# projectchrono/DEM-Engine

Measured on AMD Instinct MI355X. Metric: clump*steps/s, higher is better.
Workload: dtype f32 physics / f64 geometry

## Files before the change

### dem-engine_amd/csrc/deme_hip.hip

```cpp
#include <algorithm>
#include <cmath>
#include <cstdarg>
#include <cstdio>
#include <cstdlib>
#include <chrono>
#include <cstring>
#include <condition_variable>
#include <functional>
#include <memory>
#include <mutex>
#include <dlfcn.h>
#include <map>
#include <string>
#include <thread>
#include <vector>

#include <hip/hip_runtime.h>
#include <rocprim/rocprim.hpp>
template <unsigned RB, unsigned IPT = 8>
using DemeRadixCfg = rocprim::radix_sort_config<rocprim::default_config, rocprim::default_config,
                                                rocprim::radix_sort_onesweep_config<rocprim::kernel_config<1024, IPT>, rocprim::kernel_config<1024, IPT>, RB,
                                                                                    rocprim::block_radix_rank_algorithm::match>,
                                                1024 * 1024>;
#include <array>
// ... 125 lines not shown
    bool seeded = false;
    hipModule_t prescMod = nullptr;
    hipFunction_t prescFn = nullptr;
    DevBuf prescList, prescSlot, prescRec;
    DevBuf userWc[4][8];
    uint32_t nOwnerWc = 0, nGeoWc = 0;
    bool hasGhosts = false;
    uint32_t asyncLead = 0;
    DevBuf revSlot;
    const void* revAcc = nullptr;
    bool pairsOnce = false;
    PrescArgs laterPa{nullptr, nullptr};
    bool crossStale = false;
    char* pin = nullptr;
    int spinSync = 1;
    bool snapPending = false;
    DevBuf ownersSnap;
    hipStream_t detStream = nullptr;
    hipEvent_t evSnap = nullptr, evP1 = nullptr;
    uint64_t nAsyncDetections = 0;
    std::vector<uint32_t> hShared;
    DevBuf sharedIds, sharedBuf;
    bool tailFused = true;
    bool inGroupStep = false;
    hipStream_t haloStream = nullptr;
    hipEvent_t evStepDone = nullptr, evHaloDone = nullptr;
    bool overlapDetect = false;
    hipModule_t rulesMod = nullptr;
    DemeAdaptive ad{};
    hipEvent_t evDet0 = nullptr, evDet1 = nullptr, evWin0 = nullptr, evWin1 = nullptr;
// ... 67 lines not shown
}

#define HIPCK(call)                                                                                   \
    do {                                                                                              \
        hipError_t _e = (call);                                                                       \
        if (_e != hipSuccess)                                                                         \
            return fail(c, DEME_ERR_HIP, "%s failed: %s (%s:%d)", #call, hipGetErrorString(_e), __FILE__, __LINE__); \
    } while (0)

constexpr size_t PIN_BYTES = 16384;
constexpr size_t PIN_HEAVY = 0;
constexpr size_t PIN_RANGES = 128;
constexpr size_t PIN_LEGACY = 256;
constexpr size_t PIN_TRI = 384;
constexpr size_t PIN_UNIQUE = 448;
constexpr size_t PIN_DETECT = 1024;
static_assert(PIN_HEAVY + sizeof(RangeCounters) <= PIN_RANGES && PIN_RANGES + sizeof(RangeCounters) <= PIN_LEGACY &&
                  PIN_LEGACY + sizeof(RangeCounters) <= PIN_TRI && PIN_TRI + sizeof(uint32_t) <= PIN_UNIQUE &&
                  PIN_UNIQUE + sizeof(unsigned long long) <= PIN_DETECT && PIN_DETECT + sizeof(DetectHead) <= PIN_BYTES,
              "the read-back slots overlap or leave the pinned block");
static_assert(PIN_RANGES % 8 == 0 && PIN_LEGACY % 8 == 0 && PIN_TRI % 8 == 0 && PIN_UNIQUE % 8 == 0 && PIN_DETECT % 8 == 0,
              "a read-back slot is aligned for the counters it holds");
template <typename T>
static inline T* pin_at(deme_ctx* c, size_t slot) {
    return reinterpret_cast<T*>(c->pin + slot);
}
static hipError_t sync_readback(deme_ctx* c, hipStream_t st, bool spin) {
    if (c->spinSync && spin) {
        const auto t0 = std::chrono::steady_clock::now();
        for (int it = 0;; it++) {
            const hipError_t q = hipStreamQuery(st);
            if (q != hipErrorNotReady)
                return q;
            if ((it & 255) == 255 && std::chrono::steady_clock::now() - t0 > std::chrono::milliseconds(5))
                break;
        }
    }
    return hipStreamSynchronize(st);
}
template <typename T>
const T* read_back(deme_ctx* c, size_t slot, const void* dev, hipStream_t st, bool spin, size_t bytes = sizeof(T)) {
    T* host = pin_at<T>(c, slot);
    hipError_t e = hipMemcpyAsync(host, dev, bytes, hipMemcpyDeviceToHost, st);
    if (e == hipSuccess)
        e = sync_readback(c, st, spin);
    if (e == hipSuccess)
        return host;
    fail(c, DEME_ERR_HIP, "a detection's read-back failed: %s", hipGetErrorString(e));
    return nullptr;
}

int ensure(deme_ctx* c, DevBuf& b, size_t bytes, bool keep = false) {
    if (bytes <= b.bytes && b.p)
        return DEME_OK;
    size_t want = std::max<size_t>(bytes, 256);
    if (b.p)
        want = std::max(want, b.bytes + b.bytes / 4);
    void* np = nullptr;
    HIPCK(hipMalloc(&np, want));
    if (keep && b.p && b.bytes)
        HIPCK(hipMemcpyAsync(np, b.p, b.bytes, hipMemcpyDeviceToDevice, c->stream));
    if (b.p) {
        HIPCK(hipStreamSynchronize(c->stream));
        HIPCK(hipFree(b.p));
// ... 265 lines not shown
    return launch_margins(c, c->stream, c->owners.as<OwnerRec>(), drift);
}

int do_migrate(deme_ctx* c);

struct DetectRun {
    hipStream_t st;
    OwnerRec* ow;
    bool async;
    bool statusSeen = false;
    KeyArena ar{};
    bool segmented = false;
    uint32_t P = 0;
    uint32_t nStats = 0, compactBlocks = 0;
    uint64_t raw = 0, segMax = 0;
    DetectCounters hc{};
};
inline unsigned bin_id_bits(const deme_ctx* c) { return bits_for((uint64_t)c->hp.nbX * c->hp.nbY * c->hp.nbZ, 32); }

void open_key_arena(deme_ctx* c, DetectRun& d) {
    DetectBlock* blk = c->ctr.as<DetectBlock>();
    d.segmented = c->keySegMin && c->cntCap >= c->keySegMin && c->cntCap >= DEME_KEY_SEGS * 64u;
    d.ar.keys = c->keysRaw.as<uint64_t>();
    d.ar.segMask = d.segmented ? DEME_KEY_SEGS - 1u : 0u;
    d.ar.segCap = d.segmented ? (uint64_t)c->cntCap / DEME_KEY_SEGS : (uint64_t)c->cntCap;
    d.ar.ctr = d.segmented ? blk->segCtr : &blk->c.nContactsRaw;
}

const DetectHead* read_detect_counters(deme_ctx* c, DetectRun& d, size_t bytes) {
    const DetectHead* hh = read_back<DetectHead>(c, PIN_DETECT, c->ctr.p, d.st, !d.async, bytes);
    if (!hh || (!d.statusSeen && status_to_error(c, hh->c.status & ~DEME_ST_INCIDENCE)))
        return nullptr;
    d.statusSeen = true;
    d.hc = hh->c;
    return hh;
}

int detect_sphere_incidences(deme_ctx* c, DetectRun& d) {
    const uint32_t nS = c->nSpheres;
    d.P = 0;
    auto fill_incidence = [&]() {
        hipLaunchKernelGGL(k_fill_incidence, dim3(grid_for(nS)), dim3(256), 0, d.st, c->dp, c->binLo.as<uint4>(), c->binN.as<uint2>(),
                           c->binPartial.as<uint32_t>(), c->incKeys[0].as<uint32_t>(), c->incVals[0].as<uint32_t>(), (uint64_t)c->incCap);
    };
    if (nS) {
        c->geoStale = false;
        hipLaunchKernelGGL(k_sphere_prep, dim3(grid_for(nS)), dim3(256), 0, d.st, c->dp, d.ow, c->spheres.as<SphereRec>(),
                           c->geo.as<GeoRec>(), c->binLo.as<uint4>(), c->binN.as<uint2>(), c->binPartial.as<uint32_t>(), d.ar,
                           c->ctr.as<DetectCounters>(), c->sphFam.as<uint16_t>());
        hipLaunchKernelGGL(k_scan_small, dim3(1), dim3(DEME_SCAN_T), 0, d.st, c->binPartial.as<uint32_t>(), c->binPartial.as<uint32_t>(),
                           grid_for(nS), &c->ctr.as<DetectBlock>()->c.nIncidence);
        const bool early = c->incCap != 0;
        if (early)
            fill_incidence();
        if (!read_detect_counters(c, d, sizeof(DetectCounters)))
            return c->lastStatus;
        if (d.hc.status & DEME_ST_INCIDENCE)
            return fail(c, DEME_ERR_OVERFLOW,
                        "a sphere touches more than %u bins (margin far larger than the bin size): the incidence list cannot be built",
                        DEME_MAX_BINS_PER_SPHERE);
        if (d.hc.nIncidence > 0xFFFFFFFFull)
            return fail(c, DEME_ERR_OVERFLOW, "%llu bin-sphere incidences do not fit the 32-bit list offsets (use larger bins)",
                        d.hc.nIncidence);
        d.P = (uint32_t)d.hc.nIncidence;
        const bool grow = d.P > c->incCap;
        if (grow)
            if (int rc = grow_incidence_arena(c, (size_t)d.P + d.P / 4 + 1024))
                return rc;
        if (d.P && (grow || !early))
            fill_incidence();
    }
// ... 61 lines not shown
    hipLaunchKernelGGL(k_tri_fill, dim3(grid_for(nT)), dim3(256), 0, st, c->dp, nT, c->triWorld.as<TriWorld>(), c->triLo.as<int4>(),
                       c->triHi.as<int4>(), c->triOffsets.as<uint32_t>(), c->triKeys[0].as<uint32_t>(), c->triVals[0].as<uint32_t>(),
                       (uint64_t)c->triCap);
    if (int rc = with_temp(c, c->sortTmp, [&](void* tmp, size_t& bytes) {
            return rocprim::radix_sort_pairs(tmp, bytes, c->triKeys[0].as<uint32_t>(), c->triKeys[1].as<uint32_t>(),
                                             c->triVals[0].as<uint32_t>(), c->triVals[1].as<uint32_t>(), (size_t)TP, 0, bin_id_bits(c), st);
        }))
        return rc;
    hipLaunchKernelGGL(k_tri_sweep, dim3(grid_for(TP)), dim3(256), 0, st, c->dp, TP, c->triKeys[1].as<uint32_t>(),
                       c->triVals[1].as<uint32_t>(), c->triWorld.as<TriWorld>(), d.P, c->incKeys[1].as<uint32_t>(),
                       c->incVals[1].as<uint32_t>(), c->geo.as<GeoRec>(), c->sphFam.as<uint16_t>(), d.ar);
    return DEME_OK;
}
int detect_close_arena(deme_ctx* c, DetectRun& d) {
    d.compactBlocks = 0;
    if (d.segmented) {
        d.compactBlocks = (uint32_t)std::min<uint64_t>(grid_for(std::max<uint64_t>(c->lastSegMax + c->lastSegMax / 8 + 1024, 1)), grid_for(d.ar.segCap));
        hipLaunchKernelGGL(k_compact_keys, dim3(d.compactBlocks, DEME_KEY_SEGS), dim3(256), 0, d.st, c->keysRaw.as<uint64_t>(), d.ar.segCap,
                           c->ctr.as<DetectBlock>(), 0u, c->keysSorted[c->keysCur ^ 1].as<uint64_t>(), c->binStat.as<uint2>(), d.nStats);
    }
    const DetectHead* hh = read_detect_counters(c, d, d.segmented ? sizeof(DetectHead) : sizeof(DetectCounters));
    if (!hh)
        return c->lastStatus;
    d.raw = d.hc.nContactsRaw, d.segMax = 0;
    if (d.segmented) {
        d.raw = 0;
        for (uint32_t g = 0; g < DEME_KEY_SEGS; g++) {
            d.raw += hh->segCount[g];
            d.segMax = std::max<uint64_t>(d.segMax, hh->segCount[g]);
        }
    }
    return DEME_OK;
}

size_t contact_arena_wanted(uint64_t raw, uint64_t segMax, uint64_t segCap, size_t marks, size_t cap) {
    size_t grow = 0;
    if (raw > cap || segMax > segCap) {
        const size_t want = std::max<size_t>(raw, (size_t)segMax * DEME_KEY_SEGS);
        grow = want + want / 4 + 1024;
    }
    if (marks && raw + marks > std::max(cap, grow))
        grow = (size_t)raw + marks + raw / 4 + 1024;
    return grow;
}

int detect_order_keys(deme_ctx* c, DetectRun& d, uint64_t* nCout) {
    const hipStream_t st = d.st;
    const size_t nPersist = c->hPersist.size();
    uint64_t nC = d.raw + nPersist;
    const int next = c->keysCur ^ 1;
    uint64_t* rawKeys = c->keysRaw.as<uint64_t>();
    if (d.segmented) {
        c->lastSegMax = d.segMax;
        if (grid_for(d.segMax) > d.compactBlocks)
            hipLaunchKernelGGL(k_compact_keys, dim3((unsigned)grid_for(d.segMax) - d.compactBlocks, DEME_KEY_SEGS), dim3(256), 0, st,
                               c->keysRaw.as<uint64_t>(), d.ar.segCap, c->ctr.as<DetectBlock>(), d.compactBlocks,
                               c->keysSorted[next].as<uint64_t>(), (const uint2*)nullptr, 0u);
        if (d.raw)
            rawKeys = c->keysSorted[next].as<uint64_t>();
    }
    if (nPersist)
        HIPCK(hipMemcpyAsync(rawKeys + d.raw, c->persistKeys.p, nPersist * 8, hipMemcpyDeviceToDevice, st));
    if (nC) {
        const unsigned bitsA = bits_for(c->dp.nSpheres, 31);
        if (int rc = ensure(c, c->keysMid, (size_t)c->cntCap * 8))
            return rc;
        uint64_t* mid = c->keysMid.as<uint64_t>();
        if (int rc = with_temp(c, c->sortTmp, [&](void* tmp, size_t& bytes) {
                return deme_radix_sort<DemeRadixCfg<8>, false>(tmp, bytes, rawKeys, mid, nullptr, nullptr, (size_t)nC, (size_t)c->cntCap, 31,
                                                               33 + bitsA, DEME_SORT_OWN_FROM_KEYS64, st);
            }))
            return rc;
// ... 28 lines not shown
        if (int rc = detect_sphere_incidences(c, d))
            return rc;
        if (int rc = detect_sort_sweep(c, d))
            return rc;
        if (int rc = detect_triangles(c, d))
            return rc;
        if (int rc = detect_close_arena(c, d))
            return rc;
        if (const size_t cap = contact_arena_wanted(d.raw, d.segMax, d.ar.segCap, c->hPersist.size(), c->cntCap)) {
            if (async)
                HIPCK(hipStreamSynchronize(c->stream));
            if (int rc = grow_contact_arena(c, cap))
                return rc;
            continue;
        }
        c->nActiveBins = d.hc.nActiveBins;
        c->maxInBin = d.hc.maxInBin ? d.hc.maxInBin : (d.P ? 1u : 0u);
        if (c->maxInBin > c->dp.errOutBinSphNum)
            return fail(c, DEME_ERR_BIN_TOO_FULL,
                        "a bin contains %u sphere components, exceeding the allowance %u (SetMaxSphereInBin)", c->maxInBin,
                        c->dp.errOutBinSphNum);
        return detect_order_keys(c, d, nCout);
    }
    return fail(c, DEME_ERR_OVERFLOW, "contact arena kept overflowing");
}

int build_legacy_lists(deme_ctx* c, ContactList& L, const OwnerRec* ow, hipStream_t st) {
    const uint64_t nC = L.nListed;
    if (nC) {
        const unsigned obits = bits_for(c->nOwners, 32);
        if (int rc = with_temp(c, c->sortTmp, [&](void* tmp, size_t& bytes) {
                return rocprim::radix_sort_pairs(tmp, bytes, L.ownerB[0].as<uint32_t>(), L.ownerB[1].as<uint32_t>(), L.bIdx[0].as<uint32_t>(),
                                                 L.bIdx[1].as<uint32_t>(), (size_t)nC, 0, obits, st);
            }))
            return rc;
    }
    if (c->hasGhosts) {
// ... 80 lines not shown
            unsigned int* cnt = &L.rangeCtr.as<RangeCounters>()->nSM;
            if (int rc = with_temp(c, c->scanTmp, [&](void* tmp, size_t& bytes) {
                    return rocprim::select(tmp, bytes, rocprim::counting_iterator<uint32_t>(0), L.smFlag.as<uint8_t>(), L.smList.as<uint32_t>(), cnt,
                                           (size_t)nC, st);
                }))
                return rc;
        }
        hipLaunchKernelGGL(k_run_starts, dim3(grid_for(nC)), dim3(256), 0, st, (uint32_t)nC, L.ownerA.as<uint32_t>(), c->nOwners,
                           L.aStart.as<uint32_t>());
    } else {
        HIPCK(hipMemsetAsync(L.aStart.p, 0, ((size_t)c->nOwners + 1) * 4, st));
    }
    L.nListed = nC, L.listKeys = next;
    return DEME_OK;
}
int build_tiles(deme_ctx* c, ContactList& L, const OwnerRec* ow, hipStream_t st, RangeCounters& hr) {
    const uint32_t nTiles = tile_count(c);
    hipLaunchKernelGGL(k_scan_small, dim3(1), dim3(DEME_SCAN_T), 0, st, L.tileRem.as<uint32_t>(), L.tileBase.as<uint32_t>(), nTiles + 1,
                       &L.rangeCtr.as<RangeCounters>()->nRemote);
    hipLaunchKernelGGL(k_tile_build, dim3(nTiles), dim3(256), 0, st, c->dp, c->nOwners, L.info.as<uint4>(),
                       L.ownerB[0].as<uint32_t>(), L.aStart.as<uint32_t>(), ow, L.tileBase.as<uint32_t>(), L.tInfo.as<uint2>(),
                       L.hList.as<uint32_t>(), L.hCount.as<uint32_t>(),
                       c->hasGhosts ? L.tileMode.as<uint32_t>() : (uint32_t*)nullptr, L.lOff.as<uint16_t>(),
                       L.lPos.as<uint16_t>(), L.lCount.as<uint32_t>(), L.rankC.as<uint32_t>(), L.remKey[0].as<uint32_t>(),
                       L.remVal.as<uint32_t>(), L.tileOrg.as<int64_t>(), L.rangeCtr.as<RangeCounters>(), nTiles,
                       L.tileBig.as<uint32_t>(), L.bigList.as<uint32_t>(), c->recContact.as<uint32_t>());
    hipLaunchKernelGGL(k_tile_stats, dim3((nTiles + 1023u) / 1024u), dim3(256), 0, st, nTiles, L.hCount.as<uint32_t>(),
                       L.lCount.as<uint32_t>(), L.rangeCtr.as<RangeCounters>());
    const RangeCounters* got = read_back<RangeCounters>(c, PIN_RANGES, L.rangeCtr.p, st, true);
    if (!got)
        return c->lastStatus;
    hr = *got;
    const uint32_t nR = (uint32_t)hr.nRemote + hr.nExtra;
    L.nBigTiles = hr.nBig;
    const unsigned obits = bits_for(c->nOwners, 32);
    if (nR) {
        if (int rc = with_temp(c, c->sortTmp, [&](void* tmp, size_t& bytes) {
                return deme_radix_sort<DemeRadixCfg<10>, true>(tmp, bytes, L.remKey[0].as<uint32_t>(), L.remKey[1].as<uint32_t>(),
                                                               L.remVal.as<uint32_t>(), L.rIdx.as<uint32_t>(), (size_t)nR, (size_t)c->cntCap, 0, obits,
                                                               DEME_SORT_OWN_FROM_RECORDS, st);
            }))
            return rc;
        hipLaunchKernelGGL(k_run_starts, dim3(grid_for(nR)), dim3(256), 0, st, nR, L.remKey[1].as<uint32_t>(), c->nOwners,
                           L.rStart.as<uint32_t>());
    } else {
        HIPCK(hipMemsetAsync(L.rStart.p, 0, ((size_t)c->nOwners + 1) * 4, st));
    }
    hipLaunchKernelGGL(k_owner_ranges_tile, dim3(grid_for(c->nOwners)), dim3(256), 0, st, c->dp, ow, L.aStart.as<uint32_t>(),
                       L.lOff.as<uint16_t>(), L.rStart.as<uint32_t>(), L.heavy.as<uint8_t>(), L.fixedFlag.as<uint8_t>(),
                       L.heavyList.as<uint32_t>(), (uint32_t)(L.heavyList.bytes / 4), L.rangeCtr.as<RangeCounters>());
    return DEME_OK;
}
int build_closed_tiles(deme_ctx* c, ContactList& L, const OwnerRec* ow, hipStream_t st) {
    const uint32_t nTiles = tile_count(c);
    hipLaunchKernelGGL(k_in_count, dim3(grid_for((size_t)c->nOwners + 1)), dim3(256), 0, st, c->dp, ow,
                       L.rStart.as<uint32_t>(), c->inCnt.as<uint32_t>());
    if (int rc = with_temp(c, c->scanTmp, [&](void* tmp, size_t& bytes) {
            return rocprim::exclusive_scan(tmp, bytes, c->inCnt.as<uint32_t>(), c->inStart.as<uint32_t>(), 0u, (size_t)c->nOwners + 1,
                                           rocprim::plus<uint32_t>(), st);
        }))
        return rc;
    hipLaunchKernelGGL(k_tile_incoming, dim3(nTiles), dim3(256), 0, st, c->dp, c->nOwners, L.info.as<uint4>(),
// ... 13 lines not shown
}
void commit_list(deme_ctx* c, uint64_t nC) {
    c->fusedPrevValid = false;
    c->conValid = false;
    c->nPrev = c->haveList ? c->nContacts : 0;
    c->nContacts = nC;
    c->keysCur ^= 1;
    c->listSerial++;
    c->haveList = true;
    c->seeded = false;
    c->mapFresh = true;
    c->nDetections++;
}

void order_watch_drift(deme_ctx* c, const RangeCounters& hr);
int detect_part2(deme_ctx* c, ContactList& L, const OwnerRec* ow, hipStream_t st, uint64_t nC) {
    L.invalidate();
    const bool tiled = tile_eligible(c, nC);
    RangeCounters hr{};
    if (int rc = build_owner_arrays(c, L, st, nC, tiled))
        return rc;
    if (tiled) {
        if (int rc = build_tiles(c, L, ow, st, hr))
            return rc;
        if (fused_eligible(c, hr))
            if (int rc = build_closed_tiles(c, L, ow, st))
                return rc;
        if (int rc = fetch_heavy_counts(c, L, st))
            return rc;
    } else {
        if (int rc = build_legacy_lists(c, L, ow, st))
            return rc;
        if (int rc = read_legacy_counts(c, L, st, hr))
            return rc;
    }
    L.tileActive = tiled;
    L.tileMaxHalo = hr.tileMaxHalo, L.tileMaxList = hr.tileMaxList;
    L.nSA = hr.nSA;
// ... 1 lines not shown
    if (tiled)
        order_watch_drift(c, hr);
    commit_list(c, nC);
    return DEME_OK;
}


int do_detect(deme_ctx* c) {
    if (c->mapFresh)
        if (int rc = do_migrate(c))
            return rc;
    ScopedTimer tm(c, "detect", true);
    uint64_t nC = 0;
    if (int rc = detect_part1(c, c->stream, c->owners.as<OwnerRec>(), false, &nC))
        return rc;
    return detect_part2(c, c->list[c->cur], c->owners.as<OwnerRec>(), c->stream, nC);
}

int do_migrate(deme_ctx* c) {
    ContactList& L = c->list[c->cur];
    const uint32_t nW = c->hp.nContactWildcards;
    if (!c->mapFresh)
        return DEME_OK;
    c->mapFresh = false;
    if (nW == 0) {
        c->nWcStored = c->nContacts;
        return DEME_OK;
    }
    const int next = c->wcCur ^ 1;
    if (c->nContacts)
        hipLaunchKernelGGL(k_migrate, dim3(grid_for(c->nContacts)), dim3(256), 0, c->stream, (uint32_t)c->nContacts, nW,
// ... 415 lines not shown
    deme_ctx* c = new deme_ctx();
    c->device = device;
    if (hipStreamCreateWithFlags(&c->stream, hipStreamNonBlocking) != hipSuccess) {
        delete c;
        return DEME_ERR_HIP;
    }
    if (ensure(c, c->ctr, sizeof(DetectBlock)) || ensure(c, c->scanTmp, 1 << 20)) {
        delete c;
        return DEME_ERR_HIP;
    }
    hipMemsetAsync(c->ctr.p, 0, sizeof(DetectBlock), c->stream);
    if (hipHostMalloc((void**)&c->pin, PIN_BYTES, hipHostMallocDefault) != hipSuccess) {
        deme_ctx_destroy(c);
        return DEME_ERR_HIP;
    }
    if (const char* e = getenv("DEME_ARITH"))
        c->arith = (strcmp(e, "exact") == 0) ? DEME_ARITH_EXACT : DEME_ARITH_FAST;
    if (const char* e = getenv("DEME_XCD_GROUP"))
        c->xcdGroup = (uint32_t)std::max(0, atoi(e));
    if (const char* e = getenv("DEME_SPIN_SYNC"))
        c->spinSync = atoi(e);
    if (const char* e = getenv("DEME_KEY_SEG_MIN"))
        c->keySegMin = (size_t)std::max(0ll, atoll(e));
    *out = c;
    return DEME_OK;
}

void deme_ctx_destroy(deme_ctx* c) {
    if (!c)
        return;
    hipSetDevice(c->device);
    hipStreamSynchronize(c->stream);
    drain_timers(c);
    for (auto e : c->eventPool)
        hipEventDestroy(e);
    for (hipModule_t m : {c->customMod, c->prescMod, c->rulesMod})
// ... 7 lines not shown
            hipEventDestroy(e);
    if (c->haloStream) {
        hipStreamSynchronize(c->haloStream);
        hipEventDestroy(c->evStepDone);
        hipEventDestroy(c->evHaloDone);
        hipStreamDestroy(c->haloStream);
    }
    if (c->pin)
        hipHostFree(c->pin);
    for (ContactList& l : c->list)
        for (DevBuf* b : l.buffers())
            if (b->p)
                hipFree(b->p);
    if (c->hrEvent)
        hipEventDestroy(c->hrEvent);
    if (c->detStream) {
        hipStreamSynchronize(c->detStream);
        hipEventDestroy(c->evSnap);
        hipEventDestroy(c->evP1);
        hipStreamDestroy(c->detStream);
    }
    DevBuf* all[] = {&c->hCountIn, &c->ownersNext, &c->recContact, &c->inCnt, &c->inStart, &c->tInfoIn, &c->inContact,
                     &c->sphFam, &c->dO2E, &c->dS2E, &c->rec32, &c->revSlot, &c->nextAcc, &c->binStat, &c->volumes,
                     &c->persistKeys, &c->owners, &c->spheres, &c->acc, &c->conA4, &c->conA2, &c->conB4, &c->conB2, &c->aSum,
                     &c->prescList, &c->prescSlot, &c->prescRec, &c->tris, &c->triWorld, &c->triLo, &c->triHi, &c->triCounts,
                     &c->triOffsets, &c->triKeys[0], &c->triKeys[1], &c->triVals[0], &c->triVals[1], &c->comp, &c->massProps,
                     &c->anal, &c->matPair, &c->E, &c->nu, &c->CoR, &c->mu, &c->Crr, &c->famMasks, &c->famExtra, &c->famFlags,
                     &c->geo, &c->binLo, &c->binN, &c->binPartial, &c->incKeys[0], &c->incKeys[1], &c->incVals[0],
                     &c->incVals[1], &c->keysRaw, &c->keysSorted[0], &c->keysSorted[1], &c->wc[0], &c->wc[1], &c->ctr,
                     &c->scanTmp, &c->sortTmp, &c->rec[0], &c->rec[1], &c->rec[2], &c->rec[3], &c->stage, &c->sharedIds,
// ... 762 lines not shown
        return DEME_OK;
    if (int rc = ensure(c, c->ownersSnap, (size_t)c->nOwners * sizeof(OwnerRec)))
        return rc;
    if (int rc = ensure(c, c->keysMid, (size_t)c->cntCap * 8))
        return rc;
    return async_size_next(c);
}
static int async_part2(deme_ctx* c, uint64_t nC) {
    ContactList& N = c->list[c->cur ^ 1];
    if (int rc = async_size_next(c))
        return rc;
    {
        ScopedTimer tm(c, "detect_async_part2", true, c->detStream);
        HIPCK(hipMemsetAsync(N.heavy.p, 0, N.heavy.bytes, c->detStream));
        HIPCK(hipMemsetAsync(N.fixedFlag.p, 0, N.fixedFlag.bytes, c->detStream));
        if (int rc = detect_part2(c, N, c->ownersSnap.as<OwnerRec>(), c->detStream, nC))
            return rc;
    }
    c->cur ^= 1;
    HIPCK(hipEventRecord(c->evP1, c->detStream));
    HIPCK(hipStreamWaitEvent(c->stream, c->evP1, 0));
    if (int rc = do_migrate(c))
        return rc;
    c->stepsSinceCD = 0;
    c->listStale = false;
    c->nAsyncDetections++;
    return DEME_OK;
}
static int async_detection_cycle(deme_ctx* c) {
    const uint32_t D = c->asyncLead;
    if (int rc = async_snapshot(c))
// ... 2473 lines not shown
```

### dem-engine_amd/csrc/deme_kernels.h

```cpp
#pragma once
#include "deme_device.h"
#include "deme_owner_cols.h"

namespace deme_dev {

#define DEME_NULL_BINID_DEV 0xFFFFFFFFu
#define DEME_ST_VELOCITY 1u
#define DEME_ST_NONFINITE 2u
#define DEME_ST_INCIDENCE 4u
#define DEME_MAX_BINS_PER_SPHERE 0xFFFFFFu

struct DetectCounters {
    unsigned long long nContactsRaw;
    unsigned int nActiveBins;
    unsigned int maxInBin;
    unsigned int status;
    unsigned int pad0;
    unsigned long long nIncidence;
    unsigned int pad[8];
};

#define DEME_KEY_SEGS 64u
#define DEME_KEY_SEG_STRIDE 16u
struct DetectBlock {
// ... 9 lines not shown
    uint64_t* keys;
    unsigned long long* ctr;
    uint64_t segCap;
    uint32_t segMask;
};
__device__ inline uint32_t arena_seg(const KeyArena& a) {
    return blockIdx.x & a.segMask;
}
__device__ inline unsigned long long arena_reserve(const KeyArena& a, uint32_t seg, unsigned long long n) {
    return atomicAdd(&a.ctr[seg * DEME_KEY_SEG_STRIDE], n);
}
__device__ inline void arena_store(const KeyArena& a, uint32_t seg, unsigned long long slot, uint64_t key) {
    if (slot < a.segCap)
        a.keys[(uint64_t)seg * a.segCap + slot] = key;
}
__device__ void bin_stats_block(const uint2* __restrict__ perBlock, uint32_t nBlocks, uint32_t block, DetectCounters* ctr);
__global__ __launch_bounds__(256) void k_compact_keys(const uint64_t* __restrict__ in, uint64_t segCap, DetectBlock* blk, uint32_t xOff,
                                                      uint64_t* __restrict__ out, const uint2* __restrict__ stats, uint32_t nStats) {
    __shared__ unsigned long long sStart, sCount;
    const uint32_t seg = blockIdx.y;
    if (threadIdx.x < 64) {
        static_assert(DEME_KEY_SEGS == 64, "one lane per segment");
        const unsigned long long raw = blk->segCtr[threadIdx.x * DEME_KEY_SEG_STRIDE];
        if (stats && seg == 0 && blockIdx.x == 0)
            blk->segCount[threadIdx.x] = raw;
        const unsigned long long cnt = min(raw, (unsigned long long)segCap);
        unsigned long long inc = cnt;
        for (int d = 1; d < 64; d <<= 1) {
            const unsigned long long u = __shfl_up(inc, d);
            if ((int)threadIdx.x >= d)
                inc += u;
        }
        if (threadIdx.x == seg)
            sStart = inc - cnt, sCount = cnt;
    }
    __syncthreads();
    const uint64_t i = ((uint64_t)xOff + blockIdx.x) * blockDim.x + threadIdx.x;
    if (i < sCount)
        out[sStart + i] = in[(uint64_t)seg * segCap + i];
    if (stats && seg == 0)
// ... 130 lines not shown
                    unsigned long long slot0 = 0;
                    if ((int)lane == leader)
                        slot0 = arena_reserve(ar, arena_seg(ar), (unsigned long long)__popcll(m));
                    slot0 = __shfl(slot0, leader);
                    const unsigned long long slot = slot0 + (unsigned long long)__popcll(m & ((1ull << lane) - 1ull));
                    if (hit)
                        arena_store(ar, arena_seg(ar), slot, make_key(DEME_KEY_CLASS_SA, s, ob0 + k));
                }
            }
        }
    }
}

#define DEME_SCAN_T 1024u
#define DEME_SCAN_IPT 4u
__global__ __launch_bounds__(DEME_SCAN_T) void k_scan_small(const uint32_t* in, uint32_t* out, uint32_t n, unsigned long long* totalOut) {
    __shared__ unsigned long long sWave[DEME_SCAN_T / 64];
    __shared__ unsigned long long sCarry;
    const uint32_t lane = threadIdx.x & 63u, w = threadIdx.x >> 6;
    if (threadIdx.x == 0)
        sCarry = 0;
    __syncthreads();
    for (uint32_t base = 0; base < n; base += DEME_SCAN_T * DEME_SCAN_IPT) {
        const uint32_t first = base + threadIdx.x * DEME_SCAN_IPT;
        uint32_t v[DEME_SCAN_IPT];
        unsigned long long sum = 0;
#pragma unroll
        for (uint32_t i = 0; i < DEME_SCAN_IPT; i++) {
            v[i] = first + i < n ? in[first + i] : 0u;
            sum += v[i];
        }
// ... 13 lines not shown
            total += t;
        }
#pragma unroll
        for (uint32_t i = 0; i < DEME_SCAN_IPT; i++) {
            if (first + i < n)
                out[first + i] = (uint32_t)run;
            run += v[i];
        }
        __syncthreads();
        if (threadIdx.x == 0)
            sCarry += total;
        __syncthreads();
    }
    if (threadIdx.x == 0)
        *totalOut = sCarry;
}

__global__ __launch_bounds__(256) void k_fill_incidence(const DevParams p, const uint4* __restrict__ binLo,
                                                        const uint2* __restrict__ binN,
                                                        const uint32_t* __restrict__ partialPrefix,
                                                        uint32_t* __restrict__ keys, uint32_t* __restrict__ vals,
                                                        uint64_t cap) {
    __shared__ uint32_t sWaveSum[4];
    const uint32_t s = blockIdx.x * blockDim.x + threadIdx.x;
    const bool valid = s < p.nSpheres;
    const uint4 lo = valid ? binLo[s] : make_uint4(0u, 0u, 0u, 0u);
    const uint2 n = valid ? binN[s] : make_uint2(0u, 0u);
    const uint64_t n64 = (uint64_t)lo.w * n.x * n.y;
    const uint32_t cnt = n64 > DEME_MAX_BINS_PER_SPHERE ? 0u : (uint32_t)n64;
    const uint32_t lane = threadIdx.x & 63u, w = threadIdx.x >> 6;
// ... 854 lines not shown
}

#define DEME_HEAVY_THRESHOLD 256u
struct RangeCounters {
    unsigned int nHeavy;
    unsigned int nHeavyFree;
    unsigned int nSA, nSM;
    unsigned int tileOverflow;
    unsigned int tileMaxHalo, tileMaxList;
    unsigned int nBig;
    unsigned int nExtra;
    unsigned int tileHaloSum;
    unsigned int nBigIn;
    unsigned int tileMaxHaloIn;
    unsigned long long nRemote;
    unsigned int pad[2];
};

__global__ __launch_bounds__(256) void k_run_starts(uint32_t n, const uint32_t* __restrict__ owner, uint32_t nOwners,
                                                    uint32_t* __restrict__ start) {
    const uint32_t i = blockIdx.x * blockDim.x + threadIdx.x;
    if (i >= n)
        return;
    const uint32_t cur = owner[i];
    const uint32_t first = (i == 0) ? 0u : owner[i - 1] + 1u;
    for (uint32_t o = first; o <= cur && o <= nOwners; o++)
        start[o] = i;
    if (i == n - 1)
        for (uint32_t o = cur + 1; o <= nOwners; o++)
            start[o] = n;
}

// ... 462 lines not shown
```

### dem-engine_amd/csrc/deme_tile.h

```cpp
#pragma once
#include "deme_force_fast.h"

#ifndef DEME_TILE_NB
#define DEME_TILE_NB 128
#endif
#ifndef DEME_TILE_HMAX
#define DEME_TILE_HMAX 192
#endif
#ifndef DEME_TILE_T
#define DEME_TILE_T 256
#endif
#define DEME_TILE_HP2 256
#define DEME_TILE_LREG 4
#define DEME_TILE_LMAX (DEME_TILE_LREG * DEME_TILE_T)
static_assert(DEME_TILE_T >= 2 * DEME_TILE_NB, "one pulling thread per owner and side");
static_assert(DEME_TILE_NB + DEME_TILE_HMAX <= 2 * DEME_TILE_T, "a thread stages at most two owner records");
static_assert(DEME_TILE_LMAX == DEME_TILE_LREG * DEME_TILE_T, "list entries per thread");
#define DEME_TILE_HASH 1024u
#ifndef DEME_TILE_REC
#define DEME_TILE_REC 6
#endif
#define DEME_TILE_REC_USER 5
#ifndef DEME_JIT_NW
#define DEME_JIT_NW 1
// ... 925 lines not shown
            while (j > b && lp[j - 1] > v) {
                lp[j] = lp[j - 1];
                j--;
            }
            lp[j] = v;
        }
    }
    __syncthreads();
    for (uint32_t i = tid; i < nLoc; i += 256)
        lPos[c0 + i] = lp[i];
    for (uint32_t i = tid; i <= DEME_TILE_NB; i += 256)
        lOff[(size_t)t * (DEME_TILE_NB + 1) + i] = (uint16_t)off[i];
}

__global__ __launch_bounds__(256) void k_tile_stats(uint32_t nTiles, const uint32_t* __restrict__ hCount,
                                                    const uint32_t* __restrict__ lCount, RangeCounters* rc) {
    __shared__ uint32_t mh[4], ml[4], sh[4];
    uint32_t a = 0, b = 0, sum = 0;
    for (uint32_t k = 0; k < 4; k++) {
        const uint32_t t = (blockIdx.x * 4u + k) * 256u + threadIdx.x;
        if (t < nTiles)
            a = max(a, hCount[t]), b = max(b, lCount[t]), sum += hCount[t];
    }
    for (int o = 32; o > 0; o >>= 1) {
        a = max(a, (uint32_t)__shfl_xor((int)a, o));
        b = max(b, (uint32_t)__shfl_xor((int)b, o));
        sum += (uint32_t)__shfl_xor((int)sum, o);
    }
    if ((threadIdx.x & 63u) == 0)
        mh[threadIdx.x >> 6] = a, ml[threadIdx.x >> 6] = b, sh[threadIdx.x >> 6] = sum;
    __syncthreads();
    if (threadIdx.x == 0) {
        atomicAdd(&rc->tileHaloSum, sh[0] + sh[1] + sh[2] + sh[3]);
        atomicMax(&rc->tileMaxHalo, max(max(mh[0], mh[1]), max(mh[2], mh[3])));
        atomicMax(&rc->tileMaxList, max(max(ml[0], ml[1]), max(ml[2], ml[3])));
    }
}

__global__ __launch_bounds__(256) void k_owner_ranges_tile(const DevParams p, const OwnerRec* __restrict__ owners,
                                                           const uint32_t* __restrict__ aStart, const uint16_t* __restrict__ lOff,
                                                           const uint32_t* __restrict__ rStart, uint8_t* __restrict__ heavy,
                                                           uint8_t* __restrict__ fixedFlag, uint32_t* __restrict__ heavyList,
                                                           uint32_t heavyCap, RangeCounters* rc) {
    const uint32_t o = blockIdx.x * blockDim.x + threadIdx.x;
    if (o >= p.nOwners)
        return;
    const uint32_t t = o / DEME_TILE_NB, k = o - t * DEME_TILE_NB;
    const uint16_t* lo = lOff + (size_t)t * (DEME_TILE_NB + 1);
    const uint32_t nA = aStart[o + 1] - aStart[o], nB = (uint32_t)(lo[k + 1] - lo[k]) + (rStart[o + 1] - rStart[o]);
    const uint32_t fw = owners[o].family;
// ... 19 lines not shown
```

Before: 6.520 billion.

## Post detection counters to pinned host mailboxes instead of stream-sync read-backs

Kernels now write small counter payloads plus a stamped flag straight into pinned host memory (system-scope release stores), and the host spins on that flag instead of issuing a memcpy and synchronizing the stream. It also starts the remote-record sort speculatively from the mailed count when the last detection had no big tiles, and defers the bin-stat read-back behind an event so key ordering can be enqueued first. This is meant to cut host-device round-trip latency on the contact-detection critical path. The cost is more complex ordering logic, a last-block ticket in k_tile_stats, and a fallback path when the mail times out.

```diff
diff --git a/dem-engine_amd/csrc/deme_hip.hip b/dem-engine_amd/csrc/deme_hip.hip
--- a/dem-engine_amd/csrc/deme_hip.hip
+++ b/dem-engine_amd/csrc/deme_hip.hip
@@ -163,6 +163,11 @@
     bool crossStale = false;
     char* pin = nullptr;
     int spinSync = 1;
+    int mailbox = 1;
+    char* pinDev = nullptr;
+    uint32_t mailStamp = 0;
+    hipEvent_t statEvent = nullptr;
+    int lastBigTiles = -1;
     bool snapPending = false;
     DevBuf ownersSnap;
     hipStream_t detStream = nullptr;
@@ -260,13 +265,28 @@
 constexpr size_t PIN_LEGACY = 256;
 constexpr size_t PIN_TRI = 384;
 constexpr size_t PIN_UNIQUE = 448;
+constexpr size_t PIN_BINSTAT = 512;
 constexpr size_t PIN_DETECT = 1024;
+constexpr size_t mail_bytes(size_t payload) { return payload + 8; }
+struct SegCounts {
+    unsigned long long n[DEME_KEY_SEGS];
+};
+constexpr size_t PIN_MAIL_INC = 640;
+constexpr size_t PIN_MAIL_REMOTE = 768;
+constexpr size_t PIN_MAIL_RANGES = 896;
+constexpr size_t PIN_MAIL_KEYS = 2048;
 static_assert(PIN_HEAVY + sizeof(RangeCounters) <= PIN_RANGES && PIN_RANGES + sizeof(RangeCounters) <= PIN_LEGACY &&
                   PIN_LEGACY + sizeof(RangeCounters) <= PIN_TRI && PIN_TRI + sizeof(uint32_t) <= PIN_UNIQUE &&
-                  PIN_UNIQUE + sizeof(unsigned long long) <= PIN_DETECT && PIN_DETECT + sizeof(DetectHead) <= PIN_BYTES,
+                  PIN_UNIQUE + sizeof(unsigned long long) <= PIN_BINSTAT && PIN_BINSTAT + sizeof(DetectCounters) <= PIN_MAIL_INC &&
+                  PIN_MAIL_INC + mail_bytes(8) <= PIN_MAIL_REMOTE && PIN_MAIL_REMOTE + mail_bytes(8) <= PIN_MAIL_RANGES &&
+                  PIN_MAIL_RANGES + mail_bytes(sizeof(RangeCounters)) <= PIN_DETECT && PIN_DETECT + sizeof(DetectHead) <= PIN_MAIL_KEYS &&
+                  PIN_MAIL_KEYS + mail_bytes(sizeof(SegCounts)) <= PIN_BYTES,
               "the read-back slots overlap or leave the pinned block");
-static_assert(PIN_RANGES % 8 == 0 && PIN_LEGACY % 8 == 0 && PIN_TRI % 8 == 0 && PIN_UNIQUE % 8 == 0 && PIN_DETECT % 8 == 0,
+static_assert(PIN_RANGES % 8 == 0 && PIN_LEGACY % 8 == 0 && PIN_TRI % 8 == 0 && PIN_UNIQUE % 8 == 0 && PIN_DETECT % 8 == 0 &&
+                  PIN_BINSTAT % 8 == 0,
               "a read-back slot is aligned for the counters it holds");
+static_assert(PIN_MAIL_INC % 128 == 0 && PIN_MAIL_REMOTE % 128 == 0 && PIN_MAIL_RANGES % 128 == 0 && PIN_MAIL_KEYS % 128 == 0,
+              "a mail slot starts a cache line: the host polls it while copies land in the slots beside it");
 template <typename T>
 static inline T* pin_at(deme_ctx* c, size_t slot) {
     return reinterpret_cast<T*>(c->pin + slot);
@@ -294,6 +314,62 @@
         return host;
     fail(c, DEME_ERR_HIP, "a detection's read-back failed: %s", hipGetErrorString(e));
     return nullptr;
+}
+
+struct MailReq {
+    unsigned long long* dev = nullptr;
+    uint32_t stamp = 0;
+    bool on = false;
+};
+static MailReq mail_request(deme_ctx* c, size_t slot, bool on) {
+    MailReq m;
+    if (!on)
+        return m;
+    m.on = true;
+    if (++c->mailStamp == 0)
+        ++c->mailStamp;
+    m.stamp = c->mailStamp;
+    if (c->mailbox != 2)
+        m.dev = reinterpret_cast<unsigned long long*>(c->pinDev + slot);
+    return m;
+}
+#ifdef DEME_MAIL_TIMES
+#define DEME_MAIL_TIMED(c, slot, t0)                                                                                                     \
+    fprintf(stderr, "mail_wait slot %zu: %.1f us\n", (size_t)(slot),                                                                       \
+            std::chrono::duration<double, std::micro>(std::chrono::steady_clock::now() - (t0)).count())
+#else
+#define DEME_MAIL_TIMED(c, slot, t0) (void)0
+#endif
+template <typename T>
+const T* mail_wait(deme_ctx* c, size_t slot, uint32_t stamp, hipStream_t st, uint32_t* small = nullptr) {
+    static_assert(sizeof(T) % 8 == 0, "a mail payload is whole words of 8 bytes");
+    const uint64_t* word = pin_at<uint64_t>(c, slot + sizeof(T));
+    auto arrived = [&]() {
+        const uint64_t w = __atomic_load_n(word, __ATOMIC_ACQUIRE);
+        if ((uint32_t)(w >> 32) != stamp)
+            return false;
+        if (small)
+            *small = (uint32_t)w;
+        return true;
+    };
+    const auto t0 = std::chrono::steady_clock::now();
+    int asked = 0;
+    for (int it = 0;; it++) {
+        if (arrived()) {
+            DEME_MAIL_TIMED(c, slot, t0);
+            return pin_at<T>(c, slot);
+        }
+        if ((it & 255) == 255) {
+            const auto ms = std::chrono::duration_cast<std::chrono::milliseconds>(std::chrono::steady_clock::now() - t0).count();
+            if (ms >= 5)
+                return nullptr;
+            if (ms > asked) {
+                asked = (int)ms;
+                if (hipStreamQuery(st) != hipErrorNotReady)
+                    return arrived() ? pin_at<T>(c, slot) : nullptr;
+            }
+        }
+    }
 }
 
 int ensure(deme_ctx* c, DevBuf& b, size_t bytes, bool keep = false) {
@@ -589,8 +665,10 @@
     uint32_t P = 0;
     uint32_t nStats = 0, compactBlocks = 0;
     uint64_t raw = 0, segMax = 0;
+    bool statsPending = false;
     DetectCounters hc{};
 };
+inline bool mail_on(const deme_ctx* c, const DetectRun& d) { return c->mailbox && c->spinSync && !d.async; }
 inline unsigned bin_id_bits(const deme_ctx* c) { return bits_for((uint64_t)c->hp.nbX * c->hp.nbY * c->hp.nbZ, 32); }
 
 void open_key_arena(deme_ctx* c, DetectRun& d) {
@@ -602,13 +680,30 @@
     d.ar.ctr = d.segmented ? blk->segCtr : &blk->c.nContactsRaw;
 }
 
+int take_status(deme_ctx* c, DetectRun& d, uint32_t status) {
+    if (!d.statusSeen)
+        if (int rc = status_to_error(c, status & ~DEME_ST_INCIDENCE))
+            return rc;
+    d.statusSeen = true;
+    return DEME_OK;
+}
 const DetectHead* read_detect_counters(deme_ctx* c, DetectRun& d, size_t bytes) {
     const DetectHead* hh = read_back<DetectHead>(c, PIN_DETECT, c->ctr.p, d.st, !d.async, bytes);
-    if (!hh || (!d.statusSeen && status_to_error(c, hh->c.status & ~DEME_ST_INCIDENCE)))
+    if (!hh || take_status(c, d, hh->c.status))
         return nullptr;
-    d.statusSeen = true;
     d.hc = hh->c;
     return hh;
+}
+int read_incidence_total(deme_ctx* c, DetectRun& d, const MailReq& m) {
+    uint32_t status = 0;
+    if (m.on)
+        if (const unsigned long long* total = mail_wait<unsigned long long>(c, PIN_MAIL_INC, m.stamp, d.st, &status)) {
+            if (int rc = take_status(c, d, status))
+                return rc;
+            d.hc.nIncidence = *total, d.hc.status = status;
+            return DEME_OK;
+        }
+    return read_detect_counters(c, d, sizeof(DetectCounters)) ? DEME_OK : (int)c->lastStatus;
 }
 
 int detect_sphere_incidences(deme_ctx* c, DetectRun& d) {
@@ -623,13 +718,15 @@
         hipLaunchKernelGGL(k_sphere_prep, dim3(grid_for(nS)), dim3(256), 0, d.st, c->dp, d.ow, c->spheres.as<SphereRec>(),
                            c->geo.as<GeoRec>(), c->binLo.as<uint4>(), c->binN.as<uint2>(), c->binPartial.as<uint32_t>(), d.ar,
                            c->ctr.as<DetectCounters>(), c->sphFam.as<uint16_t>());
+        const MailReq mail = mail_request(c, PIN_MAIL_INC, mail_on(c, d));
         hipLaunchKernelGGL(k_scan_small, dim3(1), dim3(DEME_SCAN_T), 0, d.st, c->binPartial.as<uint32_t>(), c->binPartial.as<uint32_t>(),
-                           grid_for(nS), &c->ctr.as<DetectBlock>()->c.nIncidence);
+                           grid_for(nS), &c->ctr.as<DetectBlock>()->c.nIncidence, mail.dev, mail.stamp,
+                           (const DetectCounters*)c->ctr.as<DetectCounters>());
         const bool early = c->incCap != 0;
         if (early)
             fill_incidence();
-        if (!read_detect_counters(c, d, sizeof(DetectCounters)))
-            return c->lastStatus;
+        if (int rc = read_incidence_total(c, d, mail))
+            return rc;
         if (d.hc.status & DEME_ST_INCIDENCE)
             return fail(c, DEME_ERR_OVERFLOW,
                         "a sphere touches more than %u bins (margin far larger than the bin size): the incidence list cannot be built",
@@ -721,22 +818,55 @@
 }
 int detect_close_arena(deme_ctx* c, DetectRun& d) {
     d.compactBlocks = 0;
+    d.statsPending = false;
+    MailReq mail;
     if (d.segmented) {
+        mail = mail_request(c, PIN_MAIL_KEYS, mail_on(c, d) && d.statusSeen);
         d.compactBlocks = (uint32_t)std::min<uint64_t>(grid_for(std::max<uint64_t>(c->lastSegMax + c->lastSegMax / 8 + 1024, 1)), grid_for(d.ar.segCap));
         hipLaunchKernelGGL(k_compact_keys, dim3(d.compactBlocks, DEME_KEY_SEGS), dim3(256), 0, d.st, c->keysRaw.as<uint64_t>(), d.ar.segCap,
-                           c->ctr.as<DetectBlock>(), 0u, c->keysSorted[c->keysCur ^ 1].as<uint64_t>(), c->binStat.as<uint2>(), d.nStats);
-    }
-    const DetectHead* hh = read_detect_counters(c, d, d.segmented ? sizeof(DetectHead) : sizeof(DetectCounters));
-    if (!hh)
-        return c->lastStatus;
+                           c->ctr.as<DetectBlock>(), 0u, c->keysSorted[c->keysCur ^ 1].as<uint64_t>(), c->binStat.as<uint2>(), d.nStats,
+                           mail.dev, mail.stamp);
+        if (mail.on) {
+            HIPCK(hipMemcpyAsync(pin_at<DetectCounters>(c, PIN_BINSTAT), c->ctr.p, sizeof(DetectCounters), hipMemcpyDeviceToHost, d.st));
+            HIPCK(hipEventRecord(c->statEvent, d.st));
+            d.statsPending = true;
+        }
+    }
+    const unsigned long long* seg = nullptr;
+    if (mail.on)
+        if (const SegCounts* sc = mail_wait<SegCounts>(c, PIN_MAIL_KEYS, mail.stamp, d.st))
+            seg = sc->n;
+    if (!seg) {
+        const DetectHead* hh = read_detect_counters(c, d, d.segmented ? sizeof(DetectHead) : sizeof(DetectCounters));
+        if (!hh)
+            return c->lastStatus;
+        seg = hh->segCount;
+    }
     d.raw = d.hc.nContactsRaw, d.segMax = 0;
     if (d.segmented) {
         d.raw = 0;
         for (uint32_t g = 0; g < DEME_KEY_SEGS; g++) {
-            d.raw += hh->segCount[g];
-            d.segMax = std::max<uint64_t>(d.segMax, hh->segCount[g]);
+            d.raw += seg[g];
+            d.segMax = std::max<uint64_t>(d.segMax, seg[g]);
         }
     }
+    return DEME_OK;
+}
+int take_bin_stats(deme_ctx* c, DetectRun& d) {
+    hipError_t e = hipErrorNotReady;
+    const auto t0 = std::chrono::steady_clock::now();
+    for (int it = 0; e == hipErrorNotReady; it++) {
+        e = hipEventQuery(c->statEvent);
+        if ((it & 255) == 255 && std::chrono::steady_clock::now() - t0 > std::chrono::milliseconds(5))
+            break;
+    }
+    if (e == hipErrorNotReady)
+        e = hipEventSynchronize(c->statEvent);
+    if (e != hipSuccess)
+        return fail(c, DEME_ERR_HIP, "a detection's read-back failed: %s", hipGetErrorString(e));
+    const DetectCounters* s = pin_at<DetectCounters>(c, PIN_BINSTAT);
+    d.hc.nActiveBins = s->nActiveBins, d.hc.maxInBin = s->maxInBin;
+    d.statsPending = false;
     return DEME_OK;
 }
 
@@ -762,7 +892,7 @@
         if (grid_for(d.segMax) > d.compactBlocks)
             hipLaunchKernelGGL(k_compact_keys, dim3((unsigned)grid_for(d.segMax) - d.compactBlocks, DEME_KEY_SEGS), dim3(256), 0, st,
                                c->keysRaw.as<uint64_t>(), d.ar.segCap, c->ctr.as<DetectBlock>(), d.compactBlocks,
-                               c->keysSorted[next].as<uint64_t>(), (const uint2*)nullptr, 0u);
+                               c->keysSorted[next].as<uint64_t>(), (const uint2*)nullptr, 0u, (unsigned long long*)nullptr, 0u);
         if (d.raw)
             rawKeys = c->keysSorted[next].as<uint64_t>();
     }
@@ -821,13 +951,26 @@
                 return rc;
             continue;
         }
-        c->nActiveBins = d.hc.nActiveBins;
-        c->maxInBin = d.hc.maxInBin ? d.hc.maxInBin : (d.P ? 1u : 0u);
-        if (c->maxInBin > c->dp.errOutBinSphNum)
-            return fail(c, DEME_ERR_BIN_TOO_FULL,
-                        "a bin contains %u sphere components, exceeding the allowance %u (SetMaxSphereInBin)", c->maxInBin,
-                        c->dp.errOutBinSphNum);
-        return detect_order_keys(c, d, nCout);
+        auto note_bins = [&]() {
+            c->nActiveBins = d.hc.nActiveBins;
+            c->maxInBin = d.hc.maxInBin ? d.hc.maxInBin : (d.P ? 1u : 0u);
+            if (c->maxInBin > c->dp.errOutBinSphNum)
+                return fail(c, DEME_ERR_BIN_TOO_FULL,
+                            "a bin contains %u sphere components, exceeding the allowance %u (SetMaxSphereInBin)", c->maxInBin,
+                            c->dp.errOutBinSphNum);
+            return (int)DEME_OK;
+        };
+        if (!d.statsPending)
+            if (int rc = note_bins())
+                return rc;
+        if (int rc = detect_order_keys(c, d, nCout))
+            return rc;
+        if (d.statsPending) {
+            if (int rc = take_bin_stats(c, d))
+                return rc;
+            return note_bins();
+        }
+        return DEME_OK;
     }
     return fail(c, DEME_ERR_OVERFLOW, "contact arena kept overflowing");
 }
@@ -938,10 +1081,12 @@
     L.nListed = nC, L.listKeys = next;
     return DEME_OK;
 }
-int build_tiles(deme_ctx* c, ContactList& L, const OwnerRec* ow, hipStream_t st, RangeCounters& hr) {
+int build_tiles(deme_ctx* c, ContactList& L, const OwnerRec* ow, hipStream_t st, RangeCounters& hr, bool lockstep, bool lastFit) {
     const uint32_t nTiles = tile_count(c);
+    const bool mailOn = lockstep && c->mailbox && c->spinSync;
+    const MailReq mailRemote = mail_request(c, PIN_MAIL_REMOTE, mailOn && lastFit);
     hipLaunchKernelGGL(k_scan_small, dim3(1), dim3(DEME_SCAN_T), 0, st, L.tileRem.as<uint32_t>(), L.tileBase.as<uint32_t>(), nTiles + 1,
-                       &L.rangeCtr.as<RangeCounters>()->nRemote);
+                       &L.rangeCtr.as<RangeCounters>()->nRemote, mailRemote.dev, mailRemote.stamp, (const DetectCounters*)nullptr);
     hipLaunchKernelGGL(k_tile_build, dim3(nTiles), dim3(256), 0, st, c->dp, c->nOwners, L.info.as<uint4>(),
                        L.ownerB[0].as<uint32_t>(), L.aStart.as<uint32_t>(), ow, L.tileBase.as<uint32_t>(), L.tInfo.as<uint2>(),
                        L.hList.as<uint32_t>(), L.hCount.as<uint32_t>(),
@@ -949,27 +1094,46 @@
                        L.lPos.as<uint16_t>(), L.lCount.as<uint32_t>(), L.rankC.as<uint32_t>(), L.remKey[0].as<uint32_t>(),
                        L.remVal.as<uint32_t>(), L.tileOrg.as<int64_t>(), L.rangeCtr.as<RangeCounters>(), nTiles,
                        L.tileBig.as<uint32_t>(), L.bigList.as<uint32_t>(), c->recContact.as<uint32_t>());
+    const MailReq mailCounters = mail_request(c, PIN_MAIL_RANGES, mailOn);
     hipLaunchKernelGGL(k_tile_stats, dim3((nTiles + 1023u) / 1024u), dim3(256), 0, st, nTiles, L.hCount.as<uint32_t>(),
-                       L.lCount.as<uint32_t>(), L.rangeCtr.as<RangeCounters>());
-    const RangeCounters* got = read_back<RangeCounters>(c, PIN_RANGES, L.rangeCtr.p, st, true);
+                       L.lCount.as<uint32_t>(), L.rangeCtr.as<RangeCounters>(), mailCounters.dev, mailCounters.stamp);
+    const unsigned obits = bits_for(c->nOwners, 32);
+    auto order_records = [&](uint32_t nR) -> int {
+        if (nR) {
+            if (int rc = with_temp(c, c->sortTmp, [&](void* tmp, size_t& bytes) {
+                    return deme_radix_sort<DemeRadixCfg<10>, true>(tmp, bytes, L.remKey[0].as<uint32_t>(), L.remKey[1].as<uint32_t>(),
+                                                                   L.remVal.as<uint32_t>(), L.rIdx.as<uint32_t>(), (size_t)nR, (size_t)c->cntCap, 0,
+                                                                   obits, DEME_SORT_OWN_FROM_RECORDS, st);
+                }))
+                return rc;
+            hipLaunchKernelGGL(k_run_starts, dim3(grid_for(nR)), dim3(256), 0, st, nR, L.remKey[1].as<uint32_t>(), c->nOwners,
+                               L.rStart.as<uint32_t>());
+        } else {
+            HIPCK(hipMemsetAsync(L.rStart.p, 0, ((size_t)c->nOwners + 1) * 4, st));
+        }
+        return DEME_OK;
+    };
+    bool ordered = false;
+    uint32_t nOrdered = 0;
+    if (mailRemote.on)
+        if (const unsigned long long* nRemote = mail_wait<unsigned long long>(c, PIN_MAIL_REMOTE, mailRemote.stamp, st)) {
+            nOrdered = (uint32_t)*nRemote;
+            if (int rc = order_records(nOrdered))
+                return rc;
+            ordered = true;
+        }
+    const RangeCounters* got = mailCounters.on ? mail_wait<RangeCounters>(c, PIN_MAIL_RANGES, mailCounters.stamp, st) : nullptr;
+    if (!got)
+        got = read_back<RangeCounters>(c, PIN_RANGES, L.rangeCtr.p, st, true);
     if (!got)
         return c->lastStatus;
     hr = *got;
     const uint32_t nR = (uint32_t)hr.nRemote + hr.nExtra;
     L.nBigTiles = hr.nBig;
-    const unsigned obits = bits_for(c->nOwners, 32);
-    if (nR) {
-        if (int rc = with_temp(c, c->sortTmp, [&](void* tmp, size_t& bytes) {
-                return deme_radix_sort<DemeRadixCfg<10>, true>(tmp, bytes, L.remKey[0].as<uint32_t>(), L.remKey[1].as<uint32_t>(),
-                                                               L.remVal.as<uint32_t>(), L.rIdx.as<uint32_t>(), (size_t)nR, (size_t)c->cntCap, 0, obits,
-                                                               DEME_SORT_OWN_FROM_RECORDS, st);
-            }))
-            return rc;
-        hipLaunchKernelGGL(k_run_starts, dim3(grid_for(nR)), dim3(256), 0, st, nR, L.remKey[1].as<uint32_t>(), c->nOwners,
-                           L.rStart.as<uint32_t>());
-    } else {
-        HIPCK(hipMemsetAsync(L.rStart.p, 0, ((size_t)c->nOwners + 1) * 4, st));
-    }
+    c->lastBigTiles = (int)std::min<uint32_t>(hr.nBig, 0x7FFFFFFFu);
+    if (!ordered || nR != nOrdered)
+        if (int rc = order_records(nR))
+            return rc;
     hipLaunchKernelGGL(k_owner_ranges_tile, dim3(grid_for(c->nOwners)), dim3(256), 0, st, c->dp, ow, L.aStart.as<uint32_t>(),
                        L.lOff.as<uint16_t>(), L.rStart.as<uint32_t>(), L.heavy.as<uint8_t>(), L.fixedFlag.as<uint8_t>(),
                        L.heavyList.as<uint32_t>(), (uint32_t)(L.heavyList.bytes / 4), L.rangeCtr.as<RangeCounters>());
@@ -1013,14 +1177,17 @@
 }
 
 void order_watch_drift(deme_ctx* c, const RangeCounters& hr);
-int detect_part2(deme_ctx* c, ContactList& L, const OwnerRec* ow, hipStream_t st, uint64_t nC) {
+int detect_part2(deme_ctx* c, ContactList& L, const OwnerRec* ow, hipStream_t st, uint64_t nC, bool lockstep) {
     L.invalidate();
     const bool tiled = tile_eligible(c, nC);
+    const bool lastFit = c->lastBigTiles == 0;
+    if (!tiled)
+        c->lastBigTiles = -1;
     RangeCounters hr{};
     if (int rc = build_owner_arrays(c, L, st, nC, tiled))
         return rc;
     if (tiled) {
-        if (int rc = build_tiles(c, L, ow, st, hr))
+        if (int rc = build_tiles(c, L, ow, st, hr, lockstep, lastFit))
             return rc;
         if (fused_eligible(c, hr))
             if (int rc = build_closed_tiles(c, L, ow, st))
@@ -1052,7 +1219,7 @@
     uint64_t nC = 0;
     if (int rc = detect_part1(c, c->stream, c->owners.as<OwnerRec>(), false, &nC))
         return rc;
-    return detect_part2(c, c->list[c->cur], c->owners.as<OwnerRec>(), c->stream, nC);
+    return detect_part2(c, c->list[c->cur], c->owners.as<OwnerRec>(), c->stream, nC, true);
 }
 
 int do_migrate(deme_ctx* c) {
@@ -1498,12 +1665,20 @@
         deme_ctx_destroy(c);
         return DEME_ERR_HIP;
     }
+    memset(c->pin, 0, PIN_BYTES);
+    if (hipHostGetDevicePointer((void**)&c->pinDev, c->pin, 0) != hipSuccess ||
+        hipEventCreateWithFlags(&c->statEvent, hipEventDisableTiming) != hipSuccess) {
+        deme_ctx_destroy(c);
+        return DEME_ERR_HIP;
+    }
     if (const char* e = getenv("DEME_ARITH"))
         c->arith = (strcmp(e, "exact") == 0) ? DEME_ARITH_EXACT : DEME_ARITH_FAST;
     if (const char* e = getenv("DEME_XCD_GROUP"))
         c->xcdGroup = (uint32_t)std::max(0, atoi(e));
     if (const char* e = getenv("DEME_SPIN_SYNC"))
         c->spinSync = atoi(e);
+    if (const char* e = getenv("DEME_MAILBOX"))
+        c->mailbox = atoi(e);
     if (const char* e = getenv("DEME_KEY_SEG_MIN"))
         c->keySegMin = (size_t)std::max(0ll, atoll(e));
     *out = c;
@@ -1541,6 +1716,8 @@
                 hipFree(b->p);
     if (c->hrEvent)
         hipEventDestroy(c->hrEvent);
+    if (c->statEvent)
+        hipEventDestroy(c->statEvent);
     if (c->detStream) {
         hipStreamSynchronize(c->detStream);
         hipEventDestroy(c->evSnap);
@@ -2333,7 +2510,7 @@
         ScopedTimer tm(c, "detect_async_part2", true, c->detStream);
         HIPCK(hipMemsetAsync(N.heavy.p, 0, N.heavy.bytes, c->detStream));
         HIPCK(hipMemsetAsync(N.fixedFlag.p, 0, N.fixedFlag.bytes, c->detStream));
-        if (int rc = detect_part2(c, N, c->ownersSnap.as<OwnerRec>(), c->detStream, nC))
+        if (int rc = detect_part2(c, N, c->ownersSnap.as<OwnerRec>(), c->detStream, nC, false))
             return rc;
     }
     c->cur ^= 1;
diff --git a/dem-engine_amd/csrc/deme_kernels.h b/dem-engine_amd/csrc/deme_kernels.h
--- a/dem-engine_amd/csrc/deme_kernels.h
+++ b/dem-engine_amd/csrc/deme_kernels.h
@@ -47,16 +47,30 @@
     if (slot < a.segCap)
         a.keys[(uint64_t)seg * a.segCap + slot] = key;
 }
+__device__ inline void mail_post(unsigned long long* slot, uint32_t stamp, uint32_t n64, unsigned long long mine, uint32_t small = 0u) {
+    if (!slot)
+        return;
+    const uint32_t lane = threadIdx.x & 63u;
+    if (lane < n64)
+        slot[lane] = mine;
+    __threadfence_system();
+    if (lane == 0)
+        __hip_atomic_store(slot + n64, ((unsigned long long)stamp << 32) | small, __ATOMIC_RELEASE, __HIP_MEMORY_SCOPE_SYSTEM);
+}
+
 __device__ void bin_stats_block(const uint2* __restrict__ perBlock, uint32_t nBlocks, uint32_t block, DetectCounters* ctr);
 __global__ __launch_bounds__(256) void k_compact_keys(const uint64_t* __restrict__ in, uint64_t segCap, DetectBlock* blk, uint32_t xOff,
-                                                      uint64_t* __restrict__ out, const uint2* __restrict__ stats, uint32_t nStats) {
+                                                      uint64_t* __restrict__ out, const uint2* __restrict__ stats, uint32_t nStats,
+                                                      unsigned long long* mail, uint32_t stamp) {
     __shared__ unsigned long long sStart, sCount;
     const uint32_t seg = blockIdx.y;
     if (threadIdx.x < 64) {
         static_assert(DEME_KEY_SEGS == 64, "one lane per segment");
         const unsigned long long raw = blk->segCtr[threadIdx.x * DEME_KEY_SEG_STRIDE];
-        if (stats && seg == 0 && blockIdx.x == 0)
+        if (stats && seg == 0 && blockIdx.x == 0) {
+            mail_post(mail, stamp, DEME_KEY_SEGS, raw);
             blk->segCount[threadIdx.x] = raw;
+        }
         const unsigned long long cnt = min(raw, (unsigned long long)segCap);
         unsigned long long inc = cnt;
         for (int d = 1; d < 64; d <<= 1) {
@@ -217,7 +231,8 @@
 
 #define DEME_SCAN_T 1024u
 #define DEME_SCAN_IPT 4u
-__global__ __launch_bounds__(DEME_SCAN_T) void k_scan_small(const uint32_t* in, uint32_t* out, uint32_t n, unsigned long long* totalOut) {
+__global__ __launch_bounds__(DEME_SCAN_T) void k_scan_small(const uint32_t* in, uint32_t* out, uint32_t n, unsigned long long* totalOut,
+                                                            unsigned long long* mail, uint32_t stamp, const DetectCounters* ctr) {
     __shared__ unsigned long long sWave[DEME_SCAN_T / 64];
     __shared__ unsigned long long sCarry;
     const uint32_t lane = threadIdx.x & 63u, w = threadIdx.x >> 6;
@@ -261,6 +276,8 @@
     }
     if (threadIdx.x == 0)
         *totalOut = sCarry;
+    if (threadIdx.x < 64)
+        mail_post(mail, stamp, 1u, sCarry, mail && ctr ? ctr->status : 0u);
 }
 
 __global__ __launch_bounds__(256) void k_fill_incidence(const DevParams p, const uint4* __restrict__ binLo,
@@ -1145,8 +1162,10 @@
     unsigned int nBigIn;
     unsigned int tileMaxHaloIn;
     unsigned long long nRemote;
-    unsigned int pad[2];
+    unsigned int statsTicket;
+    unsigned int pad;
 };
+static_assert(sizeof(RangeCounters) == 64, "k_tile_stats posts the counters as 8 words of 8 bytes");
 
 __global__ __launch_bounds__(256) void k_run_starts(uint32_t n, const uint32_t* __restrict__ owner, uint32_t nOwners,
                                                     uint32_t* __restrict__ start) {
diff --git a/dem-engine_amd/csrc/deme_tile.h b/dem-engine_amd/csrc/deme_tile.h
--- a/dem-engine_amd/csrc/deme_tile.h
+++ b/dem-engine_amd/csrc/deme_tile.h
@@ -963,7 +963,8 @@
 }
 
 __global__ __launch_bounds__(256) void k_tile_stats(uint32_t nTiles, const uint32_t* __restrict__ hCount,
-                                                    const uint32_t* __restrict__ lCount, RangeCounters* rc) {
+                                                    const uint32_t* __restrict__ lCount, RangeCounters* rc, unsigned long long* mail,
+                                                    uint32_t stamp) {
     __shared__ uint32_t mh[4], ml[4], sh[4];
     uint32_t a = 0, b = 0, sum = 0;
     for (uint32_t k = 0; k < 4; k++) {
@@ -983,6 +984,19 @@
         atomicAdd(&rc->tileHaloSum, sh[0] + sh[1] + sh[2] + sh[3]);
         atomicMax(&rc->tileMaxHalo, max(max(mh[0], mh[1]), max(mh[2], mh[3])));
         atomicMax(&rc->tileMaxList, max(max(ml[0], ml[1]), max(ml[2], ml[3])));
+    }
+    if (mail && threadIdx.x < 64) {
+        uint32_t last = 0;
+        if (threadIdx.x == 0) {
+            __threadfence();
+            last = atomicAdd(&rc->statsTicket, 1u) == gridDim.x - 1u ? 1u : 0u;
+        }
+        last = (uint32_t)__shfl((int)last, 0);
+        __threadfence();
+        if (last)
+            mail_post(mail, stamp, (uint32_t)(sizeof(RangeCounters) / 8),
+                      __hip_atomic_load(reinterpret_cast<unsigned long long*>(rc) + (threadIdx.x & 7u), __ATOMIC_RELAXED,
+                                        __HIP_MEMORY_SCOPE_AGENT));
     }
 }
 
```

Result: no change. 6.572 billion, median of 6 (+0.8%).
